# naver/deep-image-retrieval

Measured on AMD Instinct MI355X. Metric: images/sec descriptor extraction (resnet101-GeM, 1024x1024), higher is better.
Workload: dtype fp16p

## Files before the change

### deep-image-retrieval_amd/csrc/conv_igemm.hip

```cpp
#include "dir_common.h"
#include "conv_device.h"
#include "conv_igemm.h"

#include <stdlib.h>
#include <string.h>
#include <algorithm>

namespace dir {

template <class DT, int BM, int BN, int WGM, int WGN, int NST, int BK, bool CIN16, bool SPLITK>
__global__ void __launch_bounds__(64 * WGM * WGN) conv_igemm_kernel(const ConvArgs a) {
    static_assert(NST >= 2 && NST <= 8, "ring depth");
    static_assert((BK == 64 || BK == 32) && (!CIN16 || BK == 64), "K-step");
    constexpr int RB = BK * 2;
    constexpr int CPR = BK / 8;
    constexpr int KS = BK / 16;
    constexpr int NT = 64 * WGM * WGN;
    constexpr int TM = BM / WGM / 32;
    constexpr int TN = BN / WGN / 32;
    constexpr int NA = BM * CPR / NT;
    constexpr int NB = BN * CPR / NT;
    constexpr int LPS = NA + NB;
    static_assert(TM >= 1 && TN >= 1, "wave tile");
    static_assert(NA >= 1 && NB >= 1 && (BM * CPR) % NT == 0 && (BN * CPR) % NT == 0, "chunk split");
// ... 354 lines not shown
    DIR_VARIANT(256, 256, 4, 2, 4, 32, "256x256_w4x2_s4_k32"),
    DIR_VARIANT(256, 256, 4, 2, 3, 32, "256x256_w4x2_s3_k32"),
    DIR_VARIANT(256, 128, 4, 2, 4, 32, "256x128_w4x2_s4_k32"),
    DIR_VARIANT(128, 128, 2, 2, 4, 32, "128x128_w2x2_s4_k32"),
    DIR_VARIANT(256, 128, 4, 2, 3, 32, "256x128_w4x2_s3_k32"),
    DIR_VARIANT(128, 256, 2, 4, 3, 32, "128x256_w2x4_s3_k32"),
    DIR_VARIANT(128, 256, 2, 2, 3, 32, "128x256_w2x2_s3_k32"),
    DIR_VARIANT(128, 128, 2, 2, 3, 32, "128x128_w2x2_s3_k32"),
    DIR_VARIANT(256, 256, 4, 4, 2, 64, "256x256_w4x4"),
    DIR_VARIANT_SK(64, 64, 2, 2, 8, 64, "64x64_w2x2_s8"),
    DIR_VARIANT_SK(64, 64, 2, 2, 4, 64, "64x64_w2x2_s4"),
    DIR_ROW("256x64_patch3x3", 256, 64, 256, 3, 64, patch3x3_admissible<64>, conv_patch3x3_launch),
    DIR_ROW("256x128_patch3x3", 256, 128, 512, 3, 64, patch3x3_admissible<128>, conv_patch3x3_launch),
    DIR_ROW("256x64_patchlc3x3", 256, 64, 512, 2, 64, conv_patch64_lc_admissible, conv_patch64_lc_launch),
    DIR_ROW("256x256_patch3x3s", 256, 256, 512, 2, 64, conv_patch3x3s_admissible, conv_patch3x3s_launch),
    DIR_ROW("512x128_patch3x3w", 512, 128, 512, 3, 32, conv_patch3x3w_admissible, conv_patch3x3w_launch),
    DIR_ROW("256x128_patchs2", 256, 128, 768, 2, 32, conv_patch3x3s2_admissible, conv_patch3x3s2_launch),
    DIR_ROW("256x256_persist1x1", 256, 256, 512, 2, 64, conv1x1_persist_admissible, conv1x1_persist_launch),
    DIR_ROW_DUAL("256x256_persist1x1_x3", 256, 256, 512, 3, 64, conv1x1_persist_x3_admissible, conv1x1_persist_x3_launch,
                 conv1x1_persist_dual_admissible, conv1x1_persist_dual_launch),
#ifdef DIR_EXPERIMENTS
    DIR_ROW("128x256_ring1x1", 128, 256, 512, 3, 64, conv1x1_ring_admissible, conv1x1_ring_launch),
#endif
    DIR_ROW("64x512_wreg1x1", 64, 512, 512, 2, 64, conv1x1_wreg_admissible, conv1x1_wreg_launch),
    DIR_ROW("64x64_small_s8", 64, 64, 512, 8, 64, conv_small_admissible, conv_small_s8_launch),
    DIR_ROW("64x64_small_s4", 64, 64, 512, 4, 64, conv_small_admissible, conv_small_s4_launch),
    DIR_ROW("64x64_small_s4k2", 64, 64, 512, 4, 64, conv_small_k2_admissible, conv_small_s4k2_launch),
    DIR_ROW_DUAL("256x256_lc1x1", 256, 256, 768, 3, 64, conv1x1_lc_plain_admissible, conv1x1_lc_launch,
                 conv1x1_lc_admissible, conv1x1_lc_dual_launch),
    DIR_ROW_DUAL("64x256_wregd1x1", 64, 256, 512, 2, 64, nullptr, nullptr, conv1x1_wregd_admissible, conv1x1_wregd_launch),
};
static constexpr int kNumVariants = sizeof(kVariants) / sizeof(kVariants[0]);

int conv_variant_count() { return kNumVariants; }
const ConvVariant& conv_variant(int i) { return kVariants[i]; }

bool conv_variant_admissible(int v, const ConvArgs& a) {
    return v >= 0 && v < kNumVariants && kVariants[v].admissible != nullptr && kVariants[v].admissible(a);
}

template <class DT>
__global__ void conv_splitk_finalize_kernel(const float* __restrict__ partial, const float* __restrict__ bias,
                                            const uint16_t* res, uint16_t* y,
                                            long total8, int Cout, long MC, int ksplit, int relu, int* ovf_flag) {
    const long i8 = (long)blockIdx.x * blockDim.x + threadIdx.x;
    if (i8 >= total8) return;
    const long o = i8 * 8;
    const int n = (int)(o % Cout);
    float v[8];
    const f32x4_t b0 = *(const DIR_GLOBAL f32x4_t*)(bias + n), b1 = *(const DIR_GLOBAL f32x4_t*)(bias + n + 4);
#pragma unroll
    for (int e = 0; e < 4; ++e) v[e] = b0[e], v[4 + e] = b1[e];
    for (int z = 0; z < ksplit; ++z) {
        const float* p = partial + (size_t)z * MC + o;
        const f32x4_t p0 = *(const DIR_GLOBAL f32x4_t*)p, p1 = *(const DIR_GLOBAL f32x4_t*)(p + 4);
#pragma unroll
        for (int e = 0; e < 4; ++e) v[e] += p0[e], v[4 + e] += p1[e];
    }
    if (res) {
        const u32x4_t rv = gload16(res + o);
#pragma unroll
        for (int e = 0; e < 4; ++e) {
            float lo, hi;
            DT::unpack(rv[e], lo, hi);
            v[2 * e] += lo;
            v[2 * e + 1] += hi;
        }
    }
    if (relu) relu8(v);
    const u32x4_t ov = pack8<DT>(v);
    gstore16(y + o, ov);
    Ovf<DT> ovf;
    ovf.see(ov);
    ovf.flush(ovf_flag);
}

int conv_launch(const ConvArgs& a, int dtype, int variant, hipStream_t stream) {
    if (a.Cout % 64 != 0) return fail(DIR_ERR_INVALID, "conv: Cout must be a multiple of 64");
    const bool cin16 = (a.Cin == 16);
    if (cin16) {
        if (a.R != 4 || a.S != 4 || a.stride != 1)
            return fail(DIR_ERR_INVALID, "conv: Cin == 16 is only the 4x4 s1 space-to-depth stem");
    } else if (a.Cin % 64 != 0) {
        return fail(DIR_ERR_INVALID, "conv: Cin must be a multiple of 64 (or 16 for the stem)");
    }
    if (a.R > 4 || a.S > 4) return fail(DIR_ERR_INVALID, "conv: filter larger than 4x4");
    if ((long)a.B * a.H * a.W * a.Cin >= (1L << 30) || (long)a.M * a.Cout >= (1L << 30) ||
        (long)a.Cout * a.Ktot >= (1L << 30))
        return fail(DIR_ERR_INVALID, "conv: tensor exceeds 2^31 bytes; lower the batch");
    if (((uintptr_t)a.x & 15) || ((uintptr_t)a.w & 15) || ((uintptr_t)a.y & 15) ||
        ((uintptr_t)a.res & 15) || ((uintptr_t)a.bias & 15))
        return fail(DIR_ERR_INVALID, "conv: tensors must be 16-byte aligned");
    if (dtype != DIR_BF16 && dtype != DIR_FP16) return fail(DIR_ERR_INVALID, "conv: bad dtype");
    if (a.x2) {
        if (variant < 0) variant = conv_pick_dual_variant(a);
        if (variant < 0 || variant >= kNumVariants || kVariants[variant].launch_dual == nullptr ||
            !kVariants[variant].admissible_dual(a) || a.R != 1 || a.S != 1 || a.stride != 1 || a.res || a.ksplit > 1 ||
            a.Cin2 % 64 != 0 || a.Ktot != a.Cin + a.Cin2 || ((uintptr_t)a.x2 & 15) ||
            (long)a.B * a.H2 * a.W2 * a.Cin2 >= (1L << 30))
            return fail(DIR_ERR_INVALID, "conv: no two-source form for this shape / variant");
        hipError_t e = kVariants[variant].launch_dual(a, dtype, stream);
        if (e != hipSuccess)
            return fail(DIR_ERR_HIP, std::string("conv launch ") + kVariants[variant].name + "/dual: " + hipGetErrorString(e));
        return DIR_OK;
    }
    if (variant < 0) variant = conv_pick_variant(a);
    if (!conv_variant_admissible(variant, a))
        return fail(DIR_ERR_INVALID, "conv: variant not admissible for this shape");
    const ConvVariant& cv = kVariants[variant];
    if (a.ksplit > 1) {
        if (!cv.has_splitk || cin16)
            return fail(DIR_ERR_INVALID, "conv: this variant has no split-K form");
        if (!a.partial || ((uintptr_t)a.partial & 15))
            return fail(DIR_ERR_INVALID, "conv: split-K needs a 16-byte aligned fp32 scratch buffer");
        if (a.ksplit > a.Ktot / cv.BK) return fail(DIR_ERR_INVALID, "conv: more K slices than K-steps");
    }
    hipError_t e = cv.launch(a, dtype, stream);
    if (e != hipSuccess)
        return fail(DIR_ERR_HIP, std::string("conv launch ") + cv.name + ": " + hipGetErrorString(e));
    if (a.ksplit > 1) {
        const long MC = (long)a.M * a.Cout, total8 = MC / 8;
        const dim3 grid((unsigned)((total8 + 255) / 256));
        if (dtype == DIR_BF16)
            hipLaunchKernelGGL(conv_splitk_finalize_kernel<BF16>, grid, dim3(256), 0, stream, a.partial, a.bias,
                               a.res, a.y, total8, a.Cout, MC, a.ksplit, a.relu, a.ovf);
        else
            hipLaunchKernelGGL(conv_splitk_finalize_kernel<FP16>, grid, dim3(256), 0, stream, a.partial, a.bias,
                               a.res, a.y, total8, a.Cout, MC, a.ksplit, a.relu, a.ovf);
        e = hipGetLastError();
        if (e != hipSuccess) return fail(DIR_ERR_HIP, std::string("conv split-K finalize: ") + hipGetErrorString(e));
    }
    return DIR_OK;
}

template <class DT>
__global__ void conv_naive_kernel(const ConvArgs a) {
    const long idx = (long)blockIdx.x * blockDim.x + threadIdx.x;
    if (idx >= (long)a.M * a.Cout) return;
    const int n = (int)(idx % a.Cout);
    const int m = (int)(idx / a.Cout);
    const int OHW = a.OH * a.OW;
    const int b = m / OHW, rem = m - b * OHW, oh = rem / a.OW, ow = rem - oh * a.OW;
    float acc = 0.f;
    for (int r = 0; r < a.R; ++r) {
        const int ih = oh * a.stride - a.pad + r;
        if ((unsigned)ih >= (unsigned)a.H) continue;
        for (int s = 0; s < a.S; ++s) {
            const int iw = ow * a.stride - a.pad + s;
            if ((unsigned)iw >= (unsigned)a.W) continue;
            const uint16_t* xp = a.x + ((size_t)(b * a.H + ih) * a.W + iw) * a.Cin;
            const uint16_t* wp = a.w + (size_t)n * a.Ktot + (r * a.S + s) * a.Cin;
            for (int c = 0; c < a.Cin; ++c) acc = fmaf(DT::to_f32(xp[c]), DT::to_f32(wp[c]), acc);
        }
    }
    float v = acc + a.bias[n];
    if (a.res) v += DT::to_f32(a.res[(size_t)m * a.Cout + n]);
    if (a.relu) v = fmaxf(v, 0.f);
    a.y[(size_t)m * a.Cout + n] = DT::from_f32(v);
}

int conv_launch_naive(const ConvArgs& a, int dtype, hipStream_t stream) {
    const long total = (long)a.M * a.Cout;
    const int threads = 256;
    const long blocks = (total + threads - 1) / threads;
    if (blocks >= (1L << 31)) return fail(DIR_ERR_INVALID, "naive conv: too many blocks");
    if (dtype == DIR_BF16)
        hipLaunchKernelGGL(conv_naive_kernel<BF16>, dim3((unsigned)blocks), dim3(threads), 0, stream, a);
// ... 9 lines not shown
```

### deep-image-retrieval_amd/csrc/conv_patchw.hip

```cpp
#include "dir_common.h"
#include "conv_device.h"
#include "conv_igemm.h"

#ifndef DIR_PATCHW_ABL
#define DIR_PATCHW_ABL 0
#endif

namespace dir {

template <class DT>
__global__ void __launch_bounds__(512) conv_patch3x3w_kernel(const ConvArgs a) {
    constexpr int TH = 16, TW = 32, PH = TH + 2, PW = TW + 2, PP = PH * PW;
    constexpr int NTH = 512, BN = 128;
    constexpr int NPL = (PP * 4 + NTH - 1) / NTH;
    constexpr int PLANE_BYTES = NPL * NTH * 16;
    constexpr int TN = 4, TMR = 2;
    constexpr int WSTAGE = 3 * BN * 64, NBW = WSTAGE / (NTH * 16);
    constexpr int NBW_X = (DIR_PATCHW_ABL & 16) ? 2 : 0;
    constexpr int NPL_X = (DIR_PATCHW_ABL & 32) ? 7 : 0;
    constexpr int NSTW = 3;
    constexpr int WOFF = 2 * PLANE_BYTES;
    constexpr int EROW = TN * 128 + 16;
    typedef typename DT::frag_t frag_t;
    static_assert(WOFF + NSTW * WSTAGE <= 160 * 1024 && NBW * NTH * 16 == WSTAGE, "LDS map");

    extern __shared__ __attribute__((aligned(16))) char smem[];

    const int tid = threadIdx.x;
    const int lane = tid & 63;
    const int wave = __builtin_amdgcn_readfirstlane(tid >> 6);
    const int lrow = lane & 31, lhi = lane >> 5;

    const int NQ = a.Cin / 32;
    const int NS = NQ * 3;
    const int tiles_n = a.Cout / BN;
    const int tiles_x = (a.OW + TW - 1) / TW;
    const int tiles_y = (a.OH + TH - 1) / TH;
    int wg = xcd_remap(blockIdx.x, gridDim.x);
    const int tile_n = wg % tiles_n;
    wg /= tiles_n;
    const int tx = wg % tiles_x;
    wg /= tiles_x;
    const int ty = wg % tiles_y;
    const int b = wg / tiles_y;
    const int oy0 = ty * TH, ox0 = tx * TW;

    const __amdgpu_buffer_rsrc_t rsrc_x = buffer_rsrc(a.x, a.x_bytes);
    const __amdgpu_buffer_rsrc_t rsrc_w = buffer_rsrc(a.w, a.w_bytes);

    uint32_t pvoff[NPL];
#pragma unroll
    for (int i = 0; i < NPL; ++i) {
        const int P = i * NTH + tid;
        const int p = P >> 2, pos = P & 3;
        const int py = p / PW, px = p - py * PW;
        const int iy = oy0 - 1 + py, ix = ox0 - 1 + px;
        const bool ok = p < PP && (unsigned)iy < (unsigned)a.H && (unsigned)ix < (unsigned)a.W;
        pvoff[i] = ok ? (uint32_t)((((b * a.H + iy) * a.W + ix) * a.Cin + ((pos ^ ((p >> 2) & 3)) << 3)) * 2) : kOOB;
    }
    auto issue_plane = [&](int q) {
        if (DIR_PATCHW_ABL & 64) return;
        char* dst = smem + (q & 1) * PLANE_BYTES;
#pragma unroll
        for (int i = 0; i < NPL; ++i) dma16(rsrc_x, dst + (i * NTH + wave * 64) * 16, pvoff[i], q * 64);
#pragma unroll
        for (int rep = 0; rep < NPL_X; ++rep)
#pragma unroll
            for (int i = 0; i < NPL; ++i) dma16(rsrc_x, dst + (i * NTH + wave * 64) * 16, pvoff[i], q * 64);
    };
    uint32_t wvoff[NBW];
#pragma unroll
    for (int i = 0; i < NBW; ++i) {
        const int L = i * NTH + tid;
        const int s = L >> 9, n = (L & 511) >> 2, pos = L & 3;
        wvoff[i] = (uint32_t)((((tile_n * BN + n) * 9 + s) * a.Cin + ((pos ^ ((n >> 2) & 3)) << 3)) * 2);
    }
    auto issue_w = [&](int sigma, int slot) {
        if (DIR_PATCHW_ABL & 64) return;
        const int q = sigma / 3, r = sigma - q * 3;
        char* dst = smem + WOFF + slot * WSTAGE;
#pragma unroll
        for (int i = 0; i < NBW; ++i) dma16(rsrc_w, dst + (i * NTH + wave * 64) * 16, wvoff[i], (r * 3 * a.Cin + q * 32) * 2);
#pragma unroll
        for (int i = 0; i < NBW_X; ++i)
            dma16(rsrc_w, dst + (i * NTH + wave * 64) * 16, wvoff[i], (((r + 1) % 3) * 3 * a.Cin + q * 32) * 2);
    };

    f32x16_t acc[TN][TMR];
#pragma unroll
    for (int i = 0; i < TN; ++i)
#pragma unroll
        for (int g = 0; g < 4; ++g) {
            const f32x4_t b4 = *(const DIR_GLOBAL f32x4_t*)(a.bias + tile_n * BN + i * 32 + 8 * g + 4 * lhi);
#pragma unroll
            for (int j = 0; j < TMR; ++j)
#pragma unroll
                for (int e = 0; e < 4; ++e) acc[i][j][4 * g + e] = b4[e];
        }

    int woffk[2];
#pragma unroll
    for (int kk = 0; kk < 2; ++kk) woffk[kk] = lrow * 64 + (((2 * kk + lhi) ^ ((lrow >> 2) & 3)) << 4);

    issue_plane(0);
    issue_w(0, 0);
    issue_w(1, 1);
    int q = 0, r = 0;
    int slot_c = 0;
    bool plane_before = false;
    for (int sigma = 0; sigma < NS; ++sigma) {
        if (((DIR_PATCHW_ABL & 4) && sigma == 0) || (DIR_PATCHW_ABL & 64)) {
        } else if (sigma + 1 >= NS) {
            asm volatile("s_waitcnt vmcnt(0)" ::: "memory");
        } else if (plane_before) {
            asm volatile("s_waitcnt vmcnt(%0)" ::"i"(NPL * (1 + NPL_X) + NBW + NBW_X) : "memory");
        } else {
            asm volatile("s_waitcnt vmcnt(%0)" ::"i"(NBW + NBW_X) : "memory");
        }
        ring_barrier();
        plane_before = false;
        if (r == 0 && q + 1 < NQ) {
            issue_plane(q + 1);
            plane_before = true;
        }
        if (sigma + 2 < NS) {
            int slot_n = slot_c + 2;
            if (slot_n >= NSTW) slot_n -= NSTW;
            issue_w(sigma + 2, slot_n);
        }
        const char* plane = smem + (q & 1) * PLANE_BYTES;
        const char* wst = smem + WOFF + slot_c * WSTAGE;
#pragma unroll
        for (int s = 0; s < ((DIR_PATCHW_ABL & 128) ? 0 : 3); ++s) {
            frag_t xf[TMR][2], wf[2][TN];
#pragma unroll
            for (int j = 0; j < TMR; ++j) {
                const int p = (wave * TMR + j + r) * PW + s + lrow;
                const int swz = (p >> 2) & 3;
#pragma unroll
                for (int kk = 0; kk < 2; ++kk) xf[j][kk] = *(const frag_t*)(plane + p * 64 + (((2 * kk + lhi) ^ swz) << 4));
            }
#pragma unroll
            for (int kk = 0; kk < 2; ++kk)
#pragma unroll
                for (int i = 0; i < TN; ++i) wf[kk][i] = *(const frag_t*)(wst + s * (BN * 64) + i * 2048 + woffk[kk]);
#pragma unroll
            for (int kk = 0; kk < 2; ++kk)
#pragma unroll
                for (int i = 0; i < TN; ++i)
#pragma unroll
                    for (int j = 0; j < TMR; ++j) {
                        if ((DIR_PATCHW_ABL & 8) && !(s == 0 || (s == 1 && kk == 0 && i < 3))) continue;
                        acc[i][j] = DT::mfma32(wf[kk][i], xf[j][kk], acc[i][j]);
                    }
        }
        asm volatile("s_waitcnt lgkmcnt(0)" ::: "memory");
        if (++slot_c == NSTW) slot_c = 0;
        if (++r == 3) {
            r = 0;
            ++q;
        }
    }
    __syncthreads();
    Ovf<DT> ovf;
    if (DIR_PATCHW_ABL & 2) {
        float sum = 0.f;
#pragma unroll
        for (int i = 0; i < TN; ++i)
#pragma unroll
            for (int j = 0; j < TMR; ++j)
#pragma unroll
                for (int e = 0; e < 16; ++e) sum += acc[i][j][e];
        if (sum == 1.2345678e30f) a.y[0] = 1;
        return;
    }

    char* ebase = smem + wave * (32 * EROW);
    constexpr int LPR = TN * 4, RPP = 64 / LPR, NPASS = 32 / RPP;
    const int ecol = (lane % LPR) * 8;
    const int erow = lane / LPR;
    const int ncol = tile_n * BN + ecol;
#pragma unroll
    for (int j = 0; j < TMR; ++j) {
#pragma unroll
        for (int i = 0; i < TN; ++i)
#pragma unroll
            for (int g = 0; g < 4; ++g) {
                f32x4_t v = {acc[i][j][4 * g + 0], acc[i][j][4 * g + 1], acc[i][j][4 * g + 2], acc[i][j][4 * g + 3]};
                *(f32x4_t*)(ebase + lrow * EROW + (i * 32 + 8 * g + 4 * lhi) * 4) = v;
            }
        wave_lds_sync();
        const int oy = oy0 + wave * TMR + j;
#pragma unroll
        for (int pass = 0; pass < NPASS; ++pass) {
            const int mrow = pass * RPP + erow;
            const f32x4_t f0 = *(const f32x4_t*)(ebase + mrow * EROW + ecol * 4);
            const f32x4_t f1 = *(const f32x4_t*)(ebase + mrow * EROW + ecol * 4 + 16);
            const int ox = ox0 + mrow;
            if (oy < a.OH && ox < a.OW) {
                float v[8] = {f0[0], f0[1], f0[2], f0[3], f1[0], f1[1], f1[2], f1[3]};
                const size_t o = ((size_t)(b * a.OH + oy) * a.OW + ox) * a.Cout + ncol;
                if (a.res) {
                    const u32x4_t rv = gload16(a.res + o);
#pragma unroll
                    for (int e = 0; e < 4; ++e) {
                        float lo, hi;
                        DT::unpack(rv[e], lo, hi);
                        v[2 * e] += lo;
                        v[2 * e + 1] += hi;
                    }
                }
                if (a.relu) relu8(v);
                const u32x4_t ov = pack8<DT>(v);
                if (!(DIR_PATCHW_ABL & 1) || ov[0] == 0x12345678u) gstore16(a.y + o, ov);
                ovf.see(ov);
            }
        }
        wave_lds_sync();
    }
    ovf.flush(a.ovf);
}

template <class DT>
__global__ void __launch_bounds__(768) conv_patch3x3w_lc_kernel(const ConvArgs a) {
    constexpr int TH = 16, TW = 32, PH = TH + 2, PW = TW + 2, PP = PH * PW;
    constexpr int NLD = 256, BN = 128;
    constexpr int NPL = (PP * 4 + NLD - 1) / NLD;
    constexpr int PLANE_BYTES = NPL * NLD * 16;
    constexpr int TN = 4, TMR = 2;
    constexpr int WSTAGE = 3 * BN * 64, NBW = WSTAGE / (NLD * 16);
    constexpr int NSTW = 3;
    constexpr int WOFF = 2 * PLANE_BYTES;
    constexpr int EROW = TN * 128 + 16;
    typedef typename DT::frag_t frag_t;
    static_assert(WOFF + NSTW * WSTAGE <= 160 * 1024 && NBW * NLD * 16 == WSTAGE, "LDS map");

    extern __shared__ __attribute__((aligned(16))) char smem[];

    const int tid = threadIdx.x;
    const int lane = tid & 63;
    const int wave = __builtin_amdgcn_readfirstlane(tid >> 6);
    const int lrow = lane & 31, lhi = lane >> 5;

    const int NQ = a.Cin / 32;
    const int NS = NQ * 3;
    const int tiles_n = a.Cout / BN;
    const int tiles_x = (a.OW + TW - 1) / TW;
    const int tiles_y = (a.OH + TH - 1) / TH;
    int wg = xcd_remap(blockIdx.x, gridDim.x);
    const int tile_n = wg % tiles_n;
    wg /= tiles_n;
    const int tx = wg % tiles_x;
    wg /= tiles_x;
    const int ty = wg % tiles_y;
    const int b = wg / tiles_y;
    const int oy0 = ty * TH, ox0 = tx * TW;

    if (wave >= 8) {
        const int lt = tid - 512;
        const int lw = wave - 8;
        const __amdgpu_buffer_rsrc_t rsrc_x = buffer_rsrc(a.x, a.x_bytes);
        uint32_t pvoff[NPL];
#pragma unroll
        for (int i = 0; i < NPL; ++i) {
            const int P = i * NLD + lt;
            const int p = P >> 2, pos = P & 3;
            const int py = p / PW, px = p - py * PW;
            const int iy = oy0 - 1 + py, ix = ox0 - 1 + px;
            const bool ok = p < PP && (unsigned)iy < (unsigned)a.H && (unsigned)ix < (unsigned)a.W;
            pvoff[i] = ok ? (uint32_t)((((b * a.H + iy) * a.W + ix) * a.Cin + ((pos ^ ((p >> 2) & 3)) << 3)) * 2) : kOOB;
        }
        const bool packed = a.w_pw != nullptr;
        const __amdgpu_buffer_rsrc_t rsrc_wp = buffer_rsrc(packed ? a.w_pw : a.w, a.w_bytes);
        uint32_t wvoff[NBW];
#pragma unroll
        for (int i = 0; i < NBW; ++i) {
            const int L = i * NLD + lt;
            const int s = L >> 9, n = (L & 511) >> 2, pos = L & 3;
            wvoff[i] = packed ? (uint32_t)(L * 16) : (uint32_t)((((tile_n * BN + n) * 9 + s) * a.Cin + ((pos ^ ((n >> 2) & 3)) << 3)) * 2);
        }
        auto issue_plane = [&](int q) {
            char* dst = smem + (q & 1) * PLANE_BYTES;
#pragma unroll
            for (int i = 0; i < NPL; ++i) dma16(rsrc_x, dst + (i * NLD + lw * 64) * 16, pvoff[i], q * 64);
        };
        auto issue_w = [&](int sigma, int slot) {
            const int q = sigma / 3, r = sigma - q * 3;
            char* dst = smem + WOFF + slot * WSTAGE;
            const int soff = packed ? (tile_n * NS + sigma) * WSTAGE : (r * 3 * a.Cin + q * 32) * 2;
#pragma unroll
            for (int i = 0; i < NBW; ++i) dma16(rsrc_wp, dst + (i * NLD + lw * 64) * 16, wvoff[i], soff);
        };
        issue_plane(0);
        issue_w(0, 0);
        if (NS > 1) issue_w(1, 1);
        int q = 0, r = 0, slot_c = 0;
        bool plane_before = false;
        for (int sigma = 0; sigma < NS; ++sigma) {
            if (sigma + 1 >= NS) {
                asm volatile("s_waitcnt vmcnt(0)" ::: "memory");
            } else if (plane_before) {
                asm volatile("s_waitcnt vmcnt(%0)" ::"i"(NPL + NBW) : "memory");
            } else {
                asm volatile("s_waitcnt vmcnt(%0)" ::"i"(NBW) : "memory");
            }
            ring_barrier();
            plane_before = false;
            if (r == 0 && q + 1 < NQ) {
                issue_plane(q + 1);
                plane_before = true;
            }
            if (sigma + 2 < NS) {
                int slot_n = slot_c + 2;
                if (slot_n >= NSTW) slot_n -= NSTW;
                issue_w(sigma + 2, slot_n);
            }
            if (++slot_c == NSTW) slot_c = 0;
            if (++r == 3) {
                r = 0;
                ++q;
            }
        }
        ring_barrier();
        return;
    }

    f32x16_t acc[TN][TMR];
#pragma unroll
    for (int i = 0; i < TN; ++i)
#pragma unroll
        for (int g = 0; g < 4; ++g) {
            const f32x4_t b4 = *(const DIR_GLOBAL f32x4_t*)(a.bias + tile_n * BN + i * 32 + 8 * g + 4 * lhi);
#pragma unroll
            for (int j = 0; j < TMR; ++j)
#pragma unroll
                for (int e = 0; e < 4; ++e) acc[i][j][4 * g + e] = b4[e];
        }
    int woffk[2];
#pragma unroll
    for (int kk = 0; kk < 2; ++kk) woffk[kk] = lrow * 64 + (((2 * kk + lhi) ^ ((lrow >> 2) & 3)) << 4);
    asm volatile("s_waitcnt vmcnt(0)" ::: "memory");

    int q = 0, r = 0, slot_c = 0;
    for (int sigma = 0; sigma < NS; ++sigma) {
        ring_barrier();
        const char* plane = smem + (q & 1) * PLANE_BYTES;
        const char* wst = smem + WOFF + slot_c * WSTAGE;
#pragma unroll
        for (int s = 0; s < 3; ++s) {
#pragma unroll
            for (int kk = 0; kk < 2; ++kk) {
                frag_t xf[TMR], wf[TN];
#pragma unroll
                for (int j = 0; j < TMR; ++j) {
                    const int p = (wave * TMR + j + r) * PW + s + lrow;
                    xf[j] = *(const frag_t*)(plane + p * 64 + (((2 * kk + lhi) ^ ((p >> 2) & 3)) << 4));
                }
#pragma unroll
                for (int i = 0; i < TN; ++i) wf[i] = *(const frag_t*)(wst + s * (BN * 64) + i * 2048 + woffk[kk]);
#pragma unroll
                for (int j = 0; j < TMR; ++j)
#pragma unroll
                    for (int i = 0; i < TN; ++i) acc[i][j] = DT::mfma32(wf[i], xf[j], acc[i][j]);
            }
        }
        asm volatile("s_waitcnt lgkmcnt(0)" ::: "memory");
        if (++slot_c == NSTW) slot_c = 0;
        if (++r == 3) {
            r = 0;
            ++q;
        }
    }
    ring_barrier();
    Ovf<DT> ovf;
    char* ebase = smem + wave * (32 * EROW);
    constexpr int LPR = TN * 4, RPP = 64 / LPR, NPASS = 32 / RPP;
    const int ecol = (lane % LPR) * 8;
    const int erow = lane / LPR;
    const int ncol = tile_n * BN + ecol;
#pragma unroll
    for (int j = 0; j < TMR; ++j) {
#pragma unroll
        for (int i = 0; i < TN; ++i)
#pragma unroll
            for (int g = 0; g < 4; ++g) {
                f32x4_t v = {acc[i][j][4 * g + 0], acc[i][j][4 * g + 1], acc[i][j][4 * g + 2], acc[i][j][4 * g + 3]};
                *(f32x4_t*)(ebase + lrow * EROW + (i * 32 + 8 * g + 4 * lhi) * 4) = v;
            }
        wave_lds_sync();
        const int oy = oy0 + wave * TMR + j;
#pragma unroll
        for (int pass = 0; pass < NPASS; ++pass) {
            const int mrow = pass * RPP + erow;
            const f32x4_t f0 = *(const f32x4_t*)(ebase + mrow * EROW + ecol * 4);
            const f32x4_t f1 = *(const f32x4_t*)(ebase + mrow * EROW + ecol * 4 + 16);
            const int ox = ox0 + mrow;
            if (oy < a.OH && ox < a.OW) {
                float v[8] = {f0[0], f0[1], f0[2], f0[3], f1[0], f1[1], f1[2], f1[3]};
                const size_t o = ((size_t)(b * a.OH + oy) * a.OW + ox) * a.Cout + ncol;
                if (a.res) {
                    const u32x4_t rv = gload16(a.res + o);
#pragma unroll
                    for (int e = 0; e < 4; ++e) {
                        float lo, hi;
                        DT::unpack(rv[e], lo, hi);
                        v[2 * e] += lo;
                        v[2 * e + 1] += hi;
                    }
                }
                if (a.relu) relu8(v);
                const u32x4_t ov = pack8<DT>(v);
                gstore16(a.y + o, ov);
                ovf.see(ov);
            }
        }
        wave_lds_sync();
    }
    ovf.flush(a.ovf);
}

bool conv_patch3x3w_admissible(const ConvArgs& a) {
    return a.R == 3 && a.S == 3 && a.stride == 1 && a.pad == 1 && a.H == a.OH && a.W == a.OW && a.Cin % 32 == 0 &&
           a.Cin >= 64 && a.Cout % 128 == 0 && (size_t)a.B * a.H * a.W * a.Cin * 2 < (1ull << 31) &&
           (size_t)a.Cout * a.Ktot * 2 < (1ull << 31);
}

__global__ void __launch_bounds__(256) pack_patchw_kernel(const uint16_t* w, uint16_t* out, int Cout, int Cin) {
    const int NQ = Cin / 32;
    const long pieces = (long)Cout * 9 * Cin / 8;
    for (long i = (long)blockIdx.x * 256 + threadIdx.x; i < pieces; i += (long)gridDim.x * 256) {
        const int L = (int)(i % 1536);
        long t = i / 1536;
        const int r = (int)(t % 3);
        t /= 3;
        const int q = (int)(t % NQ);
        const int tn = (int)(t / NQ);
        const int s = L >> 9, n = (L & 511) >> 2, pos = L & 3;
        const size_t src = ((size_t)((tn * 128 + n) * 9 + r * 3 + s)) * Cin + q * 32 + ((pos ^ ((n >> 2) & 3)) << 3);
        gstore16(out + i * 8, gload16(w + src));
    }
}

hipError_t conv_patch3x3w_pack(const uint16_t* w, uint16_t* out, int Cout, int Cin, hipStream_t stream) {
    const long pieces = (long)Cout * 9 * Cin / 8;
    const int grid = (int)((pieces + 255) / 256 < 1024 ? (pieces + 255) / 256 : 1024);
    hipLaunchKernelGGL(pack_patchw_kernel, dim3(grid), dim3(256), 0, stream, w, out, Cout, Cin);
    return hipGetLastError();
}

template <class DT>
static hipError_t launch_patch_w(const ConvArgs& a, hipStream_t stream) {
    constexpr int LDS = 2 * 5 * 512 * 16 + 3 * 3 * 128 * 64;
    static_assert(LDS <= 160 * 1024 && LDS >= 8 * 32 * (4 * 128 + 16), "LDS map (the staging area aliases it)");
    ConvArgs b = a;
    conv_fill_extents(b);
    const long blocks = (long)a.B * ((a.OH + 15) / 16) * ((a.OW + 31) / 32) * (a.Cout / 128);
    if (!env().no_patchw_lc) {
        void* scratch = nullptr;
        if (!b.w_pw && env().patchw_pack) {
            if (hipError_t e = hipMallocAsync(&scratch, b.w_bytes, stream); e != hipSuccess) return e;
            if (hipError_t e = conv_patch3x3w_pack(a.w, (uint16_t*)scratch, a.Cout, a.Cin, stream); e != hipSuccess) {
                (void)hipFreeAsync(scratch, stream);
                return e;
            }
            b.w_pw = (const uint16_t*)scratch;
        }
        auto kern = conv_patch3x3w_lc_kernel<DT>;
        static std::atomic<uint64_t> attr_lc{0};
        if (hipError_t e = ensure_dynamic_lds((const void*)kern, LDS, attr_lc); e != hipSuccess) return e;
        hipLaunchKernelGGL(kern, dim3((unsigned)blocks), dim3(768), LDS, stream, b);
        hipError_t e = hipGetLastError();
        if (scratch) {
            const hipError_t f = hipFreeAsync(scratch, stream);
            if (e == hipSuccess) e = f;
        }
        return e;
    }
    auto kern = conv_patch3x3w_kernel<DT>;
    static std::atomic<uint64_t> attr_done{0};
    if (hipError_t e = ensure_dynamic_lds((const void*)kern, LDS, attr_done); e != hipSuccess) return e;
    hipLaunchKernelGGL(kern, dim3((unsigned)blocks), dim3(512), LDS, stream, b);
    return hipGetLastError();
}

hipError_t conv_patch3x3w_launch(const ConvArgs& a, int dtype, hipStream_t stream) {
    return dtype == DIR_BF16 ? launch_patch_w<BF16>(a, stream) : launch_patch_w<FP16>(a, stream);
}

}
```

### deep-image-retrieval_amd/csrc/dir_common.h

```cpp
#pragma once
#include <hip/hip_runtime.h>
#include <stdint.h>
#include <string.h>
#include <atomic>
#include <string>

#include "../../include/dir_engine.h"

namespace dir {

typedef __attribute__((ext_vector_type(8))) __bf16 bf16x8_t;
typedef __attribute__((ext_vector_type(8))) _Float16 f16x8_t;
typedef __attribute__((ext_vector_type(16))) float f32x16_t;
typedef __attribute__((ext_vector_type(4))) float f32x4_t;
typedef __attribute__((ext_vector_type(4))) uint32_t u32x4_t;
typedef __attribute__((ext_vector_type(2))) uint32_t u32x2_t;
typedef __attribute__((ext_vector_type(4))) int i32x4_t;
typedef __attribute__((ext_vector_type(16))) int i32x16_t;
typedef __attribute__((ext_vector_type(2))) float f32x2_t;
typedef __attribute__((ext_vector_type(2))) __bf16 bf16x2_t;
typedef __attribute__((ext_vector_type(2))) _Float16 f16x2_t;

#define DIR_GLOBAL __attribute__((address_space(1)))
#define DIR_LDS __attribute__((address_space(3)))

void set_error(const std::string& msg);
int fail(int code, const std::string& msg);

#define DIR_HIP_CHECK(expr)                                                                \
    do {                                                                                   \
        hipError_t _e = (expr);                                                            \
        if (_e != hipSuccess)                                                              \
            return ::dir::fail(DIR_ERR_HIP, std::string(#expr) + ": " + hipGetErrorString(_e)); \
    } while (0)

#define DIR_CHECK(expr)                  \
    do {                                 \
        const int _rc = (expr);          \
        if (_rc != DIR_OK) return _rc;   \
    } while (0)

struct Env {
    bool c3c1_off = false, c3c1_force = false;
    bool no_ds_seam = false, no_dual = false;
    bool rev_conv1 = false, rev_conv3 = false;
    bool unfused_stem = false, stem_v1 = false;
    bool no_patchlc = false, no_wreg = false, no_patchw = false, no_x3 = false, no_patchs = false;
    bool patchw_pack = false, no_patchw_pack = false;
    bool small_k2 = false;
    bool no_patchs2 = false;
    bool x3_k2048 = false;
    bool lc1x1 = false;
    bool no_c3c1lc = false;
    bool no_smallmap = false;
    bool no_wregd = false;
    bool no_patchw_lc = false;
    bool no_xcdmap = false;
    bool no_pair_patch = false, pair_acts = false;
    int pair_stages = 1;
    bool sim_v1 = false, sim_exact = false;
    bool experiments = false;
    bool no_inplace = false;
    bool seam_full_store = false;
    bool no_stem_u8 = false;
    bool stem_pair_old = false;
    bool stem_u8_prep = false;
    bool stem_u8_wg8 = false;
    int stem_u8_seg = 0;
};
const Env& env();
void reload_env();

__host__ __device__ inline uint16_t f32_to_bf16_bits(float f) {
    uint32_t u;
    memcpy(&u, &f, 4);
    if ((u & 0x7fffffffu) > 0x7f800000u) return (uint16_t)((u >> 16) | 0x40);
    u += 0x7fffu + ((u >> 16) & 1u);
    return (uint16_t)(u >> 16);
}
__host__ __device__ inline float bf16_bits_to_f32(uint16_t h) {
    uint32_t u = ((uint32_t)h) << 16;
    float f;
    memcpy(&f, &u, 4);
    return f;
}
__host__ __device__ inline uint16_t f32_to_f16_bits(float f) {
    _Float16 h = (_Float16)f;
    uint16_t b;
    memcpy(&b, &h, 2);
    return b;
}
__host__ __device__ inline float f16_bits_to_f32(uint16_t b) {
    _Float16 h;
    memcpy(&h, &b, 2);
    return (float)h;
}

struct BF16 {
    typedef bf16x8_t frag_t;
    static constexpr int kDtype = DIR_BF16;
    __host__ __device__ static inline float to_f32(uint16_t b) { return bf16_bits_to_f32(b); }
    __host__ __device__ static inline uint16_t from_f32(float f) { return f32_to_bf16_bits(f); }
    __device__ static inline f32x16_t mfma32(frag_t a, frag_t b, f32x16_t c) {
        return __builtin_amdgcn_mfma_f32_32x32x16_bf16(a, b, c, 0, 0, 0);
    }
    __device__ static inline void unpack(uint32_t w, float& lo, float& hi) {
        lo = __builtin_bit_cast(float, w << 16);
        hi = __builtin_bit_cast(float, w & 0xffff0000u);
    }
    __device__ static inline uint32_t pack(float lo, float hi) {
        const f32x2_t v = {lo, hi};
        return __builtin_bit_cast(uint32_t, __builtin_convertvector(v, bf16x2_t));
    }
};
struct FP16 {
    typedef f16x8_t frag_t;
    static constexpr int kDtype = DIR_FP16;
    __host__ __device__ static inline float to_f32(uint16_t b) { return f16_bits_to_f32(b); }
    __host__ __device__ static inline uint16_t from_f32(float f) { return f32_to_f16_bits(f); }
    __device__ static inline f32x16_t mfma32(frag_t a, frag_t b, f32x16_t c) {
        return __builtin_amdgcn_mfma_f32_32x32x16_f16(a, b, c, 0, 0, 0);
    }
    __device__ static inline void unpack(uint32_t w, float& lo, float& hi) {
        const f32x2_t v = __builtin_convertvector(__builtin_bit_cast(f16x2_t, w), f32x2_t);
        lo = v[0];
        hi = v[1];
    }
    __device__ static inline uint32_t pack(float lo, float hi) {
        const f32x2_t v = {lo, hi};
        return __builtin_bit_cast(uint32_t, __builtin_convertvector(v, f16x2_t));
    }
};

template <class DT>
__device__ inline void unpack2(uint32_t w, float& lo, float& hi) {
    lo = DT::to_f32((uint16_t)(w & 0xffffu));
    hi = DT::to_f32((uint16_t)(w >> 16));
}
template <class DT>
__device__ inline uint32_t pack2(float lo, float hi) {
    return (uint32_t)DT::from_f32(lo) | ((uint32_t)DT::from_f32(hi) << 16);
}

__device__ inline u32x4_t gload16(const void* p) {
    return *(const DIR_GLOBAL u32x4_t*)p;
}
__device__ inline void gstore16(void* p, u32x4_t v) {
    *(DIR_GLOBAL u32x4_t*)p = v;
}
__device__ __forceinline__ f32x4_t load4_guarded(const float* __restrict__ row, int k, int D, bool vec) {
    f32x4_t v = {0.f, 0.f, 0.f, 0.f};
    if (vec && k + 3 < D) return *(const f32x4_t*)(row + k);
#pragma unroll
    for (int e = 0; e < 4; ++e)
        if (k + e < D) v[e] = row[k + e];
    return v;
}

typedef __attribute__((ext_vector_type(2))) uint16_t u16x2_t;
template <class DT>
struct Ovf {
    uint32_t m = 0;
    __device__ inline void see(uint32_t w) {
        if constexpr (DT::kDtype == DIR_FP16) {
            uint32_t t;
            asm("v_and_b32 %1, 0x7fff7fff, %2\n\tv_pk_max_u16 %0, %0, %1" : "+v"(m), "=&v"(t) : "v"(w));
        }
    }
    __device__ inline void see(const u32x4_t& v) {
#pragma unroll
        for (int e = 0; e < 4; ++e) see(v[e]);
    }
    __device__ inline void see(const u32x2_t& v) {
        see(v[0]);
        see(v[1]);
    }
    __device__ inline void flush(int* flag) const {
        if constexpr (DT::kDtype == DIR_FP16) {
            if (flag && ((m + 0x04000400u) & 0x80008000u)) atomicOr(flag, 1);
        }
    }
};

__device__ __forceinline__ void ring_barrier() {
#ifndef DIR_EXP_NO_RING_FENCE
    __builtin_amdgcn_sched_barrier(0);
#endif
    __builtin_amdgcn_s_barrier();
#ifndef DIR_EXP_NO_RING_FENCE
    __builtin_amdgcn_sched_barrier(0);
#endif
}

__device__ inline int xcd_remap(int bid, int nwg) {
    const int q = nwg >> 3, r = nwg & 7, xcd = bid & 7;
    const int start = xcd < r ? xcd * (q + 1) : r * (q + 1) + (xcd - r) * q;
    return start + (bid >> 3);
}

inline int ceil_div(int a, int b) { return (a + b - 1) / b; }
__host__ __device__ inline int pad64(int D) { return (D + 63) & ~63; }

inline int cu_count() {
    static std::atomic<int> cached[64];
// ... 23 lines not shown
```

Measured before the change: 2446.

## Switch 3x3 patch conv kernels to 16x16x32 MFMA with direct register epilogue

Replaces the 32x32x16 MFMA tiling in both 3x3 patch conv kernels with 16x16x32 MFMA tiles. Weight rows are permuted on load so each lane's accumulator holds 8 contiguous output channels, which lets the epilogue store straight from registers and drops the LDS staging pass, its wave syncs and the final block barriers. It also relaxes the launcher to accept Cin multiples of 32 when the patch variant is forced. In exchange it issues more, smaller MFMAs and changes the LDS fragment read pattern, which could lower matrix-unit throughput or add bank conflicts.

```diff
diff --git a/deep-image-retrieval_amd/csrc/conv_igemm.hip b/deep-image-retrieval_amd/csrc/conv_igemm.hip
--- a/deep-image-retrieval_amd/csrc/conv_igemm.hip
+++ b/deep-image-retrieval_amd/csrc/conv_igemm.hip
@@ -460,7 +460,9 @@
         if (a.R != 4 || a.S != 4 || a.stride != 1)
             return fail(DIR_ERR_INVALID, "conv: Cin == 16 is only the 4x4 s1 space-to-depth stem");
     } else if (a.Cin % 64 != 0) {
-        return fail(DIR_ERR_INVALID, "conv: Cin must be a multiple of 64 (or 16 for the stem)");
+        const bool forced_plane32 = variant >= 0 && variant < kNumVariants && kVariants[variant].launch == conv_patch3x3w_launch &&
+                                    a.Cin % 32 == 0 && !a.x2 && a.ksplit <= 1;
+        if (!forced_plane32) return fail(DIR_ERR_INVALID, "conv: Cin must be a multiple of 64 (or 16 for the stem)");
     }
     if (a.R > 4 || a.S > 4) return fail(DIR_ERR_INVALID, "conv: filter larger than 4x4");
     if ((long)a.B * a.H * a.W * a.Cin >= (1L << 30) || (long)a.M * a.Cout >= (1L << 30) ||
diff --git a/deep-image-retrieval_amd/csrc/conv_patchw.hip b/deep-image-retrieval_amd/csrc/conv_patchw.hip
--- a/deep-image-retrieval_amd/csrc/conv_patchw.hip
+++ b/deep-image-retrieval_amd/csrc/conv_patchw.hip
@@ -7,6 +7,96 @@
 #endif
 
 namespace dir {
+
+__host__ __device__ inline int patchw_row_channel(int n) {
+    return (n & 0x63) | ((n & 0x0c) << 1) | ((n & 0x10) >> 2);
+}
+
+struct PatchwLane {
+    int frow;
+    int fchunk;
+    int woff;
+    int nsub;
+    __device__ __forceinline__ explicit PatchwLane(int lane) {
+        const int n = lane & 15, g = lane >> 4;
+        frow = n < 8 ? n : n ^ 4;
+        fchunk = ((g & 1) << 1) | (g >> 1);
+        woff = frow * 64 + ((fchunk ^ ((frow >> 2) & 3)) << 4);
+        nsub = 8 * (g < 2 ? g : g ^ 1);
+    }
+};
+
+typedef f32x4_t patchw_acc_t[8][2][2];
+
+template <class DT>
+__device__ __forceinline__ void patchw_init_acc(patchw_acc_t& acc, const float* bias, const PatchwLane& L) {
+#pragma unroll
+    for (int c = 0; c < 8; ++c) {
+        const f32x4_t b4 = *(const DIR_GLOBAL f32x4_t*)(bias + (c >> 1) * 32 + L.nsub + 4 * (c & 1));
+#pragma unroll
+        for (int j = 0; j < 2; ++j)
+#pragma unroll
+            for (int u = 0; u < 2; ++u) acc[c][j][u] = b4;
+    }
+}
+
+template <class DT, int ABL>
+__device__ __forceinline__ void patchw_stage(patchw_acc_t& acc, const char* plane, const char* wst, int prow, const PatchwLane& L) {
+    typedef typename DT::frag_t frag_t;
+    constexpr int PW = 34;
+    auto ldw = [&](int f) { return *(const frag_t*)(wst + (f >> 3) * (128 * 64) + (f & 7) * 1024 + L.woff); };
+    frag_t xf[2][2], wf[2][2] = {{ldw(0), ldw(1)}, {}};
+#pragma unroll
+    for (int pp = 0; pp < 12; ++pp) {
+        const int s = pp >> 2;
+        if ((pp & 3) == 0) {
+#pragma unroll
+            for (int j = 0; j < 2; ++j)
+#pragma unroll
+                for (int u = 0; u < 2; ++u) {
+                    const int p = prow + j * PW + s + 16 * u + L.frow;
+                    xf[j][u] = *(const frag_t*)(plane + p * 64 + ((L.fchunk ^ ((p >> 2) & 3)) << 4));
+                }
+        }
+        if (pp + 1 < 12) {
+            wf[(pp + 1) & 1][0] = ldw(2 * pp + 2);
+            wf[(pp + 1) & 1][1] = ldw(2 * pp + 3);
+        }
+#pragma unroll
+        for (int j = 0; j < 2; ++j)
+#pragma unroll
+            for (int u = 0; u < 2; ++u)
+#pragma unroll
+                for (int h = 0; h < 2; ++h) {
+                    const int c = (2 * pp + h) & 7;
+                    if ((ABL & 8) && !(s == 0 || (s == 1 && c < 3))) continue;
+                    acc[c][j][u] = DT::mfma16(wf[pp & 1][h], xf[j][u], acc[c][j][u]);
+                }
+    }
+}
+
+template <class DT, int ABL>
+__device__ __forceinline__ void patchw_epilogue(const ConvArgs& a, const patchw_acc_t& acc, int b, int oy, int ox, int ncol) {
+    Ovf<DT> ovf;
+#pragma unroll
+    for (int j = 0; j < 2; ++j)
+#pragma unroll
+        for (int u = 0; u < 2; ++u) {
+            if (oy + j >= a.OH || ox + 16 * u >= a.OW) continue;
+            const size_t o = ((size_t)(b * a.OH + oy + j) * a.OW + ox + 16 * u) * a.Cout + ncol;
+#pragma unroll
+            for (int p = 0; p < 4; ++p) {
+                const f32x4_t f0 = acc[2 * p][j][u], f1 = acc[2 * p + 1][j][u];
+                float v[8] = {f0[0], f0[1], f0[2], f0[3], f1[0], f1[1], f1[2], f1[3]};
+                if (a.res) add_res8<DT>(v, gload16(a.res + o + 32 * p));
+                if (a.relu) relu8(v);
+                const u32x4_t ov = pack8<DT>(v);
+                if (!(ABL & 1) || ov[0] == 0x12345678u) gstore16(a.y + o + 32 * p, ov);
+                ovf.see(ov);
+            }
+        }
+    ovf.flush(a.ovf);
+}
 
 template <class DT>
 __global__ void __launch_bounds__(512) conv_patch3x3w_kernel(const ConvArgs a) {
@@ -14,14 +104,11 @@
     constexpr int NTH = 512, BN = 128;
     constexpr int NPL = (PP * 4 + NTH - 1) / NTH;
     constexpr int PLANE_BYTES = NPL * NTH * 16;
-    constexpr int TN = 4, TMR = 2;
     constexpr int WSTAGE = 3 * BN * 64, NBW = WSTAGE / (NTH * 16);
     constexpr int NBW_X = (DIR_PATCHW_ABL & 16) ? 2 : 0;
     constexpr int NPL_X = (DIR_PATCHW_ABL & 32) ? 7 : 0;
     constexpr int NSTW = 3;
     constexpr int WOFF = 2 * PLANE_BYTES;
-    constexpr int EROW = TN * 128 + 16;
-    typedef typename DT::frag_t frag_t;
     static_assert(WOFF + NSTW * WSTAGE <= 160 * 1024 && NBW * NTH * 16 == WSTAGE, "LDS map");
 
     extern __shared__ __attribute__((aligned(16))) char smem[];
@@ -29,7 +116,7 @@
     const int tid = threadIdx.x;
     const int lane = tid & 63;
     const int wave = __builtin_amdgcn_readfirstlane(tid >> 6);
-    const int lrow = lane & 31, lhi = lane >> 5;
+    const PatchwLane L(lane);
 
     const int NQ = a.Cin / 32;
     const int NS = NQ * 3;
@@ -71,9 +158,9 @@
     uint32_t wvoff[NBW];
 #pragma unroll
     for (int i = 0; i < NBW; ++i) {
-        const int L = i * NTH + tid;
-        const int s = L >> 9, n = (L & 511) >> 2, pos = L & 3;
-        wvoff[i] = (uint32_t)((((tile_n * BN + n) * 9 + s) * a.Cin + ((pos ^ ((n >> 2) & 3)) << 3)) * 2);
+        const int P = i * NTH + tid;
+        const int s = P >> 9, n = (P & 511) >> 2, pos = P & 3;
+        wvoff[i] = (uint32_t)((((tile_n * BN + patchw_row_channel(n)) * 9 + s) * a.Cin + ((pos ^ ((n >> 2) & 3)) << 3)) * 2);
     }
     auto issue_w = [&](int sigma, int slot) {
         if (DIR_PATCHW_ABL & 64) return;
@@ -86,21 +173,8 @@
             dma16(rsrc_w, dst + (i * NTH + wave * 64) * 16, wvoff[i], (((r + 1) % 3) * 3 * a.Cin + q * 32) * 2);
     };
 
-    f32x16_t acc[TN][TMR];
-#pragma unroll
-    for (int i = 0; i < TN; ++i)
-#pragma unroll
-        for (int g = 0; g < 4; ++g) {
-            const f32x4_t b4 = *(const DIR_GLOBAL f32x4_t*)(a.bias + tile_n * BN + i * 32 + 8 * g + 4 * lhi);
-#pragma unroll
-            for (int j = 0; j < TMR; ++j)
-#pragma unroll
-                for (int e = 0; e < 4; ++e) acc[i][j][4 * g + e] = b4[e];
-        }
-
-    int woffk[2];
-#pragma unroll
-    for (int kk = 0; kk < 2; ++kk) woffk[kk] = lrow * 64 + (((2 * kk + lhi) ^ ((lrow >> 2) & 3)) << 4);
+    patchw_acc_t acc;
+    patchw_init_acc<DT>(acc, a.bias + tile_n * BN, L);
 
     issue_plane(0);
     issue_w(0, 0);
@@ -130,30 +204,7 @@
         }
         const char* plane = smem + (q & 1) * PLANE_BYTES;
         const char* wst = smem + WOFF + slot_c * WSTAGE;
-#pragma unroll
-        for (int s = 0; s < ((DIR_PATCHW_ABL & 128) ? 0 : 3); ++s) {
-            frag_t xf[TMR][2], wf[2][TN];
-#pragma unroll
-            for (int j = 0; j < TMR; ++j) {
-                const int p = (wave * TMR + j + r) * PW + s + lrow;
-                const int swz = (p >> 2) & 3;
-#pragma unroll
-                for (int kk = 0; kk < 2; ++kk) xf[j][kk] = *(const frag_t*)(plane + p * 64 + (((2 * kk + lhi) ^ swz) << 4));
-            }
-#pragma unroll
-            for (int kk = 0; kk < 2; ++kk)
-#pragma unroll
-                for (int i = 0; i < TN; ++i) wf[kk][i] = *(const frag_t*)(wst + s * (BN * 64) + i * 2048 + woffk[kk]);
-#pragma unroll
-            for (int kk = 0; kk < 2; ++kk)
-#pragma unroll
-                for (int i = 0; i < TN; ++i)
-#pragma unroll
-                    for (int j = 0; j < TMR; ++j) {
-                        if ((DIR_PATCHW_ABL & 8) && !(s == 0 || (s == 1 && kk == 0 && i < 3))) continue;
-                        acc[i][j] = DT::mfma32(wf[kk][i], xf[j][kk], acc[i][j]);
-                    }
-        }
+        if (!(DIR_PATCHW_ABL & 128)) patchw_stage<DT, DIR_PATCHW_ABL>(acc, plane, wst, (wave * 2 + r) * PW, L);
         asm volatile("s_waitcnt lgkmcnt(0)" ::: "memory");
         if (++slot_c == NSTW) slot_c = 0;
         if (++r == 3) {
@@ -161,64 +212,20 @@
             ++q;
         }
     }
-    __syncthreads();
-    Ovf<DT> ovf;
     if (DIR_PATCHW_ABL & 2) {
         float sum = 0.f;
 #pragma unroll
-        for (int i = 0; i < TN; ++i)
-#pragma unroll
-            for (int j = 0; j < TMR; ++j)
-#pragma unroll
-                for (int e = 0; e < 16; ++e) sum += acc[i][j][e];
+        for (int c = 0; c < 8; ++c)
+#pragma unroll
+            for (int j = 0; j < 2; ++j)
+#pragma unroll
+                for (int u = 0; u < 2; ++u)
+#pragma unroll
+                    for (int e = 0; e < 4; ++e) sum += acc[c][j][u][e];
         if (sum == 1.2345678e30f) a.y[0] = 1;
         return;
     }
-
-    char* ebase = smem + wave * (32 * EROW);
-    constexpr int LPR = TN * 4, RPP = 64 / LPR, NPASS = 32 / RPP;
-    const int ecol = (lane % LPR) * 8;
-    const int erow = lane / LPR;
-    const int ncol = tile_n * BN + ecol;
-#pragma unroll
-    for (int j = 0; j < TMR; ++j) {
-#pragma unroll
-        for (int i = 0; i < TN; ++i)
-#pragma unroll
-            for (int g = 0; g < 4; ++g) {
-                f32x4_t v = {acc[i][j][4 * g + 0], acc[i][j][4 * g + 1], acc[i][j][4 * g + 2], acc[i][j][4 * g + 3]};
-                *(f32x4_t*)(ebase + lrow * EROW + (i * 32 + 8 * g + 4 * lhi) * 4) = v;
-            }
-        wave_lds_sync();
-        const int oy = oy0 + wave * TMR + j;
-#pragma unroll
-        for (int pass = 0; pass < NPASS; ++pass) {
-            const int mrow = pass * RPP + erow;
-            const f32x4_t f0 = *(const f32x4_t*)(ebase + mrow * EROW + ecol * 4);
-            const f32x4_t f1 = *(const f32x4_t*)(ebase + mrow * EROW + ecol * 4 + 16);
-            const int ox = ox0 + mrow;
-            if (oy < a.OH && ox < a.OW) {
-                float v[8] = {f0[0], f0[1], f0[2], f0[3], f1[0], f1[1], f1[2], f1[3]};
-                const size_t o = ((size_t)(b * a.OH + oy) * a.OW + ox) * a.Cout + ncol;
-                if (a.res) {
-                    const u32x4_t rv = gload16(a.res + o);
-#pragma unroll
-                    for (int e = 0; e < 4; ++e) {
-                        float lo, hi;
-                        DT::unpack(rv[e], lo, hi);
-                        v[2 * e] += lo;
-                        v[2 * e + 1] += hi;
-                    }
-                }
-                if (a.relu) relu8(v);
-                const u32x4_t ov = pack8<DT>(v);
-                if (!(DIR_PATCHW_ABL & 1) || ov[0] == 0x12345678u) gstore16(a.y + o, ov);
-                ovf.see(ov);
-            }
-        }
-        wave_lds_sync();
-    }
-    ovf.flush(a.ovf);
+    patchw_epilogue<DT, DIR_PATCHW_ABL>(a, acc, b, oy0 + wave * 2, ox0 + L.frow, tile_n * BN + L.nsub);
 }
 
 template <class DT>
@@ -227,12 +234,9 @@
     constexpr int NLD = 256, BN = 128;
     constexpr int NPL = (PP * 4 + NLD - 1) / NLD;
     constexpr int PLANE_BYTES = NPL * NLD * 16;
-    constexpr int TN = 4, TMR = 2;
     constexpr int WSTAGE = 3 * BN * 64, NBW = WSTAGE / (NLD * 16);
     constexpr int NSTW = 3;
     constexpr int WOFF = 2 * PLANE_BYTES;
-    constexpr int EROW = TN * 128 + 16;
-    typedef typename DT::frag_t frag_t;
     static_assert(WOFF + NSTW * WSTAGE <= 160 * 1024 && NBW * NLD * 16 == WSTAGE, "LDS map");
 
     extern __shared__ __attribute__((aligned(16))) char smem[];
@@ -240,7 +244,7 @@
     const int tid = threadIdx.x;
     const int lane = tid & 63;
     const int wave = __builtin_amdgcn_readfirstlane(tid >> 6);
-    const int lrow = lane & 31, lhi = lane >> 5;
+    const PatchwLane L(lane);
 
     const int NQ = a.Cin / 32;
     const int NS = NQ * 3;
@@ -275,9 +279,10 @@
         uint32_t wvoff[NBW];
 #pragma unroll
         for (int i = 0; i < NBW; ++i) {
-            const int L = i * NLD + lt;
-            const int s = L >> 9, n = (L & 511) >> 2, pos = L & 3;
-            wvoff[i] = packed ? (uint32_t)(L * 16) : (uint32_t)((((tile_n * BN + n) * 9 + s) * a.Cin + ((pos ^ ((n >> 2) & 3)) << 3)) * 2);
+            const int P = i * NLD + lt;
+            const int s = P >> 9, n = (P & 511) >> 2, pos = P & 3;
+            wvoff[i] = packed ? (uint32_t)(P * 16)
+                              : (uint32_t)((((tile_n * BN + patchw_row_channel(n)) * 9 + s) * a.Cin + ((pos ^ ((n >> 2) & 3)) << 3)) * 2);
         }
         auto issue_plane = [&](int q) {
             char* dst = smem + (q & 1) * PLANE_BYTES;
@@ -321,24 +326,11 @@
                 ++q;
             }
         }
-        ring_barrier();
         return;
     }
 
-    f32x16_t acc[TN][TMR];
-#pragma unroll
-    for (int i = 0; i < TN; ++i)
-#pragma unroll
-        for (int g = 0; g < 4; ++g) {
-            const f32x4_t b4 = *(const DIR_GLOBAL f32x4_t*)(a.bias + tile_n * BN + i * 32 + 8 * g + 4 * lhi);
-#pragma unroll
-            for (int j = 0; j < TMR; ++j)
-#pragma unroll
-                for (int e = 0; e < 4; ++e) acc[i][j][4 * g + e] = b4[e];
-        }
-    int woffk[2];
-#pragma unroll
-    for (int kk = 0; kk < 2; ++kk) woffk[kk] = lrow * 64 + (((2 * kk + lhi) ^ ((lrow >> 2) & 3)) << 4);
+    patchw_acc_t acc;
+    patchw_init_acc<DT>(acc, a.bias + tile_n * BN, L);
     asm volatile("s_waitcnt vmcnt(0)" ::: "memory");
 
     int q = 0, r = 0, slot_c = 0;
@@ -346,24 +338,7 @@
         ring_barrier();
         const char* plane = smem + (q & 1) * PLANE_BYTES;
         const char* wst = smem + WOFF + slot_c * WSTAGE;
-#pragma unroll
-        for (int s = 0; s < 3; ++s) {
-#pragma unroll
-            for (int kk = 0; kk < 2; ++kk) {
-                frag_t xf[TMR], wf[TN];
-#pragma unroll
-                for (int j = 0; j < TMR; ++j) {
-                    const int p = (wave * TMR + j + r) * PW + s + lrow;
-                    xf[j] = *(const frag_t*)(plane + p * 64 + (((2 * kk + lhi) ^ ((p >> 2) & 3)) << 4));
-                }
-#pragma unroll
-                for (int i = 0; i < TN; ++i) wf[i] = *(const frag_t*)(wst + s * (BN * 64) + i * 2048 + woffk[kk]);
-#pragma unroll
-                for (int j = 0; j < TMR; ++j)
-#pragma unroll
-                    for (int i = 0; i < TN; ++i) acc[i][j] = DT::mfma32(wf[i], xf[j], acc[i][j]);
-            }
-        }
+        patchw_stage<DT, 0>(acc, plane, wst, (wave * 2 + r) * PW, L);
         asm volatile("s_waitcnt lgkmcnt(0)" ::: "memory");
         if (++slot_c == NSTW) slot_c = 0;
         if (++r == 3) {
@@ -371,52 +346,7 @@
             ++q;
         }
     }
-    ring_barrier();
-    Ovf<DT> ovf;
-    char* ebase = smem + wave * (32 * EROW);
-    constexpr int LPR = TN * 4, RPP = 64 / LPR, NPASS = 32 / RPP;
-    const int ecol = (lane % LPR) * 8;
-    const int erow = lane / LPR;
-    const int ncol = tile_n * BN + ecol;
-#pragma unroll
-    for (int j = 0; j < TMR; ++j) {
-#pragma unroll
-        for (int i = 0; i < TN; ++i)
-#pragma unroll
-            for (int g = 0; g < 4; ++g) {
-                f32x4_t v = {acc[i][j][4 * g + 0], acc[i][j][4 * g + 1], acc[i][j][4 * g + 2], acc[i][j][4 * g + 3]};
-                *(f32x4_t*)(ebase + lrow * EROW + (i * 32 + 8 * g + 4 * lhi) * 4) = v;
-            }
-        wave_lds_sync();
-        const int oy = oy0 + wave * TMR + j;
-#pragma unroll
-        for (int pass = 0; pass < NPASS; ++pass) {
-            const int mrow = pass * RPP + erow;
-            const f32x4_t f0 = *(const f32x4_t*)(ebase + mrow * EROW + ecol * 4);
-            const f32x4_t f1 = *(const f32x4_t*)(ebase + mrow * EROW + ecol * 4 + 16);
-            const int ox = ox0 + mrow;
-            if (oy < a.OH && ox < a.OW) {
-                float v[8] = {f0[0], f0[1], f0[2], f0[3], f1[0], f1[1], f1[2], f1[3]};
-                const size_t o = ((size_t)(b * a.OH + oy) * a.OW + ox) * a.Cout + ncol;
-                if (a.res) {
-                    const u32x4_t rv = gload16(a.res + o);
-#pragma unroll
-                    for (int e = 0; e < 4; ++e) {
-                        float lo, hi;
-                        DT::unpack(rv[e], lo, hi);
-                        v[2 * e] += lo;
-                        v[2 * e + 1] += hi;
-                    }
-                }
-                if (a.relu) relu8(v);
-                const u32x4_t ov = pack8<DT>(v);
-                gstore16(a.y + o, ov);
-                ovf.see(ov);
-            }
-        }
-        wave_lds_sync();
-    }
-    ovf.flush(a.ovf);
+    patchw_epilogue<DT, 0>(a, acc, b, oy0 + wave * 2, ox0 + L.frow, tile_n * BN + L.nsub);
 }
 
 bool conv_patch3x3w_admissible(const ConvArgs& a) {
@@ -436,7 +366,7 @@
         const int q = (int)(t % NQ);
         const int tn = (int)(t / NQ);
         const int s = L >> 9, n = (L & 511) >> 2, pos = L & 3;
-        const size_t src = ((size_t)((tn * 128 + n) * 9 + r * 3 + s)) * Cin + q * 32 + ((pos ^ ((n >> 2) & 3)) << 3);
+        const size_t src = ((size_t)((tn * 128 + patchw_row_channel(n)) * 9 + r * 3 + s)) * Cin + q * 32 + ((pos ^ ((n >> 2) & 3)) << 3);
         gstore16(out + i * 8, gload16(w + src));
     }
 }
@@ -451,7 +381,7 @@
 template <class DT>
 static hipError_t launch_patch_w(const ConvArgs& a, hipStream_t stream) {
     constexpr int LDS = 2 * 5 * 512 * 16 + 3 * 3 * 128 * 64;
-    static_assert(LDS <= 160 * 1024 && LDS >= 8 * 32 * (4 * 128 + 16), "LDS map (the staging area aliases it)");
+    static_assert(LDS <= 160 * 1024, "LDS map");
     ConvArgs b = a;
     conv_fill_extents(b);
     const long blocks = (long)a.B * ((a.OH + 15) / 16) * ((a.OW + 31) / 32) * (a.Cout / 128);
diff --git a/deep-image-retrieval_amd/csrc/dir_common.h b/deep-image-retrieval_amd/csrc/dir_common.h
--- a/deep-image-retrieval_amd/csrc/dir_common.h
+++ b/deep-image-retrieval_amd/csrc/dir_common.h
@@ -104,6 +104,9 @@
     __device__ static inline f32x16_t mfma32(frag_t a, frag_t b, f32x16_t c) {
         return __builtin_amdgcn_mfma_f32_32x32x16_bf16(a, b, c, 0, 0, 0);
     }
+    __device__ static inline f32x4_t mfma16(frag_t a, frag_t b, f32x4_t c) {
+        return __builtin_amdgcn_mfma_f32_16x16x32_bf16(a, b, c, 0, 0, 0);
+    }
     __device__ static inline void unpack(uint32_t w, float& lo, float& hi) {
         lo = __builtin_bit_cast(float, w << 16);
         hi = __builtin_bit_cast(float, w & 0xffff0000u);
@@ -120,6 +123,9 @@
     __host__ __device__ static inline uint16_t from_f32(float f) { return f32_to_f16_bits(f); }
     __device__ static inline f32x16_t mfma32(frag_t a, frag_t b, f32x16_t c) {
         return __builtin_amdgcn_mfma_f32_32x32x16_f16(a, b, c, 0, 0, 0);
+    }
+    __device__ static inline f32x4_t mfma16(frag_t a, frag_t b, f32x4_t c) {
+        return __builtin_amdgcn_mfma_f32_16x16x32_f16(a, b, c, 0, 0, 0);
     }
     __device__ static inline void unpack(uint32_t w, float& lo, float& hi) {
         const f32x2_t v = __builtin_convertvector(__builtin_bit_cast(f16x2_t, w), f32x2_t);
```

Result: no change. 2455 (median of 6 runs) (+0.4%).
